# nv-dvl/nerfmatch

Hardware: AMD Instinct MI355X
Metric: rays*samples/sec (higher is better)
Workload: dtype fp16x3 (fp16 MFMA on hi/lo-split fp32 operands, three products per fp32 product, fp32 accumulate; fp32 everywhere else)

## Files before the change

### nerfmatch_amd/csrc/nerf_fwd_bf16.hip

```cpp
#include "nerf_split_chain.h"

namespace {
using namespace nmbf;
using nmsample::HALF_PI_F32, nmsample::SCAN_TILE, nmsample::frustum, nmsample::ray_consts, nmsample::lift_var, nmsample::ipe_fast, nmsample::view_row_value;
using nmsample::alpha_of, nmsample::trans_factor, nmsample::sigmoid, nmsample::scan_before_barrier, nmsample::scan_after_barrier, nmsample::scan_carry;
using nmsample::first_max;
static_assert(TILE == SCAN_TILE, "the compositing scan of nerf_sample.h spans two wavefronts");

template <int PART, bool OWN>
__device__ __forceinline__ void tap_prefetch(Ctx& cx) {
  if constexpr (PART == 0) __builtin_amdgcn_s_barrier();
  const char* src = reinterpret_cast<const char*>(cx.tapw);
#pragma unroll
  for (int q = (PART == 0 ? 0 : 4); q < (PART == 0 ? 4 : 7); ++q) {
    const char* sp = src + q * 4096;
    const float* dp = q < 4 ? cx.tap_ring + q * 1024 : cx.tap_ipe + (q - 4) * 1024;
    const unsigned lds = (unsigned)__builtin_amdgcn_readfirstlane((int)(unsigned)(size_t)(const __attribute__((address_space(3))) float*)dp);
    if constexpr (OWN) {
      asm volatile("s_mov_b32 m0, %0\n\tglobal_load_lds_dwordx4 %1, off\n\tglobal_load_lds_dwordx4 %1, off offset:1024\n\t"
                   "global_load_lds_dwordx4 %1, off offset:2048\n\tglobal_load_lds_dwordx4 %1, off offset:3072"
                   :: "s"(lds), "v"(sp) : "memory");
      continue;
    }
    unsigned m0_saved;
// ... 22 lines not shown
        "v_add_f32_dpp %0, %8, %8 row_half_mirror row_mask:0xf bank_mask:0x5\n\tv_add_f32_dpp %1, %9, %9 row_half_mirror row_mask:0xf bank_mask:0x5\n\t"
        "v_add_f32_dpp %2, %10, %10 row_half_mirror row_mask:0xf bank_mask:0x5\n\tv_add_f32_dpp %3, %11, %11 row_half_mirror row_mask:0xf bank_mask:0x5\n\t"
        "v_add_f32_dpp %4, %12, %12 row_half_mirror row_mask:0xf bank_mask:0x5\n\tv_add_f32_dpp %5, %13, %13 row_half_mirror row_mask:0xf bank_mask:0x5\n\t"
        "v_add_f32_dpp %6, %14, %14 row_half_mirror row_mask:0xf bank_mask:0x5\n\tv_add_f32_dpp %7, %15, %15 row_half_mirror row_mask:0xf bank_mask:0x5\n\t"
        "v_add_f32_dpp %0, %16, %16 row_half_mirror row_mask:0xf bank_mask:0xa\n\tv_add_f32_dpp %1, %17, %17 row_half_mirror row_mask:0xf bank_mask:0xa\n\t"
        "v_add_f32_dpp %2, %18, %18 row_half_mirror row_mask:0xf bank_mask:0xa\n\tv_add_f32_dpp %3, %19, %19 row_half_mirror row_mask:0xf bank_mask:0xa\n\t"
        "v_add_f32_dpp %4, %20, %20 row_half_mirror row_mask:0xf bank_mask:0xa\n\tv_add_f32_dpp %5, %21, %21 row_half_mirror row_mask:0xf bank_mask:0xa\n\t"
        "v_add_f32_dpp %6, %22, %22 row_half_mirror row_mask:0xf bank_mask:0xa\n\tv_add_f32_dpp %7, %23, %23 row_half_mirror row_mask:0xf bank_mask:0xa"
        : "=&v"(o[0]), "=&v"(o[1]), "=&v"(o[2]), "=&v"(o[3]), "=&v"(o[4]), "=&v"(o[5]), "=&v"(o[6]), "=&v"(o[7])
        : "v"(x[0]), "v"(x[1]), "v"(x[2]), "v"(x[3]), "v"(x[4]), "v"(x[5]), "v"(x[6]), "v"(x[7]),
          "v"(y[0]), "v"(y[1]), "v"(y[2]), "v"(y[3]), "v"(y[4]), "v"(y[5]), "v"(y[6]), "v"(y[7]));
}
template <int XOR>
__device__ __forceinline__ void quad_add8(float (&v)[8]) {
  if (XOR == 1)
    asm("s_nop 1\n"
        "v_add_f32_dpp %0, %0, %0 quad_perm:[1,0,3,2] row_mask:0xf bank_mask:0xf\n\tv_add_f32_dpp %1, %1, %1 quad_perm:[1,0,3,2] row_mask:0xf bank_mask:0xf\n\t"
        "v_add_f32_dpp %2, %2, %2 quad_perm:[1,0,3,2] row_mask:0xf bank_mask:0xf\n\tv_add_f32_dpp %3, %3, %3 quad_perm:[1,0,3,2] row_mask:0xf bank_mask:0xf\n\t"
        "v_add_f32_dpp %4, %4, %4 quad_perm:[1,0,3,2] row_mask:0xf bank_mask:0xf\n\tv_add_f32_dpp %5, %5, %5 quad_perm:[1,0,3,2] row_mask:0xf bank_mask:0xf\n\t"
        "v_add_f32_dpp %6, %6, %6 quad_perm:[1,0,3,2] row_mask:0xf bank_mask:0xf\n\tv_add_f32_dpp %7, %7, %7 quad_perm:[1,0,3,2] row_mask:0xf bank_mask:0xf"
        : "+v"(v[0]), "+v"(v[1]), "+v"(v[2]), "+v"(v[3]), "+v"(v[4]), "+v"(v[5]), "+v"(v[6]), "+v"(v[7]));
  else
    asm("s_nop 1\n"
        "v_add_f32_dpp %0, %0, %0 quad_perm:[2,3,0,1] row_mask:0xf bank_mask:0xf\n\tv_add_f32_dpp %1, %1, %1 quad_perm:[2,3,0,1] row_mask:0xf bank_mask:0xf\n\t"
        "v_add_f32_dpp %2, %2, %2 quad_perm:[2,3,0,1] row_mask:0xf bank_mask:0xf\n\tv_add_f32_dpp %3, %3, %3 quad_perm:[2,3,0,1] row_mask:0xf bank_mask:0xf\n\t"
        "v_add_f32_dpp %4, %4, %4 quad_perm:[2,3,0,1] row_mask:0xf bank_mask:0xf\n\tv_add_f32_dpp %5, %5, %5 quad_perm:[2,3,0,1] row_mask:0xf bank_mask:0xf\n\t"
        "v_add_f32_dpp %6, %6, %6 quad_perm:[2,3,0,1] row_mask:0xf bank_mask:0xf\n\tv_add_f32_dpp %7, %7, %7 quad_perm:[2,3,0,1] row_mask:0xf bank_mask:0xf"
        : "+v"(v[0]), "+v"(v[1]), "+v"(v[2]), "+v"(v[3]), "+v"(v[4]), "+v"(v[5]), "+v"(v[6]), "+v"(v[7]));
}
__device__ __forceinline__ float reduce_scatter_step16(float x, float y) {
  const auto r = __builtin_amdgcn_permlane16_swap(__float_as_uint(x), __float_as_uint(y), false, false);
  return __uint_as_float(r[0]) + __uint_as_float(r[1]);
}
__device__ __forceinline__ f32x4 reduce_scatter_16pairs(const float (&s1)[64], int lane) {
  float s2[32];
#pragma unroll
  for (int b = 0; b < 4; ++b) {
    float o[8], x[8], y[8];
#pragma unroll
    for (int i = 0; i < 8; ++i) { x[i] = s1[8 * b + i]; y[i] = s1[32 + 8 * b + i]; }
    dpp_pairs8(o, x, y, true);
#pragma unroll
    for (int i = 0; i < 8; ++i) s2[8 * b + i] = o[i];
  }
  float s3[16];
#pragma unroll
  for (int b = 0; b < 2; ++b) {
    float o[8], x[8], y[8];
#pragma unroll
    for (int i = 0; i < 8; ++i) { x[i] = s2[8 * b + i]; y[i] = s2[16 + 8 * b + i]; }
    dpp_pairs8(o, x, y, false);
#pragma unroll
    for (int i = 0; i < 8; ++i) s3[8 * b + i] = o[i];
  }
  float lo8[8], hi8[8];
#pragma unroll
  for (int i = 0; i < 8; ++i) { lo8[i] = s3[i]; hi8[i] = s3[8 + i]; }
  quad_add8<2>(lo8); quad_add8<2>(hi8);
  float s4[8];
#pragma unroll
  for (int i = 0; i < 8; ++i) s4[i] = (lane & 2) ? hi8[i] : lo8[i];
  float t8[8] = {s4[0], s4[1], s4[2], s4[3], s4[4], s4[5], s4[6], s4[7]};
  quad_add8<1>(t8);
  return (lane & 1) ? f32x4{t8[4], t8[5], t8[6], t8[7]} : f32x4{t8[0], t8[1], t8[2], t8[3]};
}
__device__ __forceinline__ f32x4 reduce_scatter_32rows(float (&v)[128], int lane) {
  float s1[64];
#pragma unroll
  for (int i = 0; i < 64; ++i) s1[i] = reduce_scatter_step16(v[i], v[64 + i]);
  return reduce_scatter_16pairs(s1, lane);
}

#define NM_MLP_DONE_WAIT() __builtin_amdgcn_s_waitcnt(0x0070)
#define NM_EPI_BARRIER() asm volatile("s_waitcnt lgkmcnt(0)\n\ts_barrier" ::: "memory")
template <int P, bool TAP7 = true>
__device__ __forceinline__ void nerf_fwd_body(const NerfArgs& a) {
  constexpr bool DENS = P == 2 && !TAP7;
  __shared__ __attribute__((aligned(16))) float sm[LDS_TOTAL];
  float* const sm_small = sm + LDS_SMALL;
  float* const ring = sm + LDS_RING;
  float* const sm_ipe = sm + LDS_IPE;
  float* const sm_sigma = sm + LDS_SCR;
  float* const sm_rgb = sm_sigma + TILE;
  float* const sm_t0 = sm_rgb + 3 * TILE;
  float* const sm_t1 = sm_t0 + TILE;
  float* const sm_mean = sm_t1 + TILE;
  float* const sm_dn = sm_mean + 3 * TILE;
  float* const sm_w = sm_dn + TILE;
  float* const sm_misc = sm_w + TILE;
  float* const sm_part = sm_misc + 32;
  float* const sm_feat = sm + LDS_FEAT;
  float* const sm_ex = sm + LDS_EX;
  int* const sm_lray = reinterpret_cast<int*>(sm + LDS_LEFT);
  float* const sm_lT = sm + LDS_LEFT + TILE;
  unsigned* const sm_rng = reinterpret_cast<unsigned*>(sm + LDS_RNG);

  const int tid = threadIdx.x, lane = tid & 63, wave = tid >> 6, s = lane & 31, hi = lane >> 5;
  const bool tail_ok = a.left && !(a.tail_viol && *a.tail_viol != 0);
  const int S = a.S, R = a.R;
  const int Sa = tail_ok ? a.Sa : S;
  const int left = tail_ok ? 1 : 0;
  const int ntiles = tail_ok ? a.ntiles : a.ntiles_full;
  const int SP = Sa < TILE ? Sa : TILE;
  const int nr = TILE / SP;
  const int nchunks = (Sa + TILE - 1) / TILE;
  const bool need_rgb = !(a.flags & NM_NERF_SKIP_RGB);
  const bool feat_max = (a.flags & NM_NERF_FEAT_MAX) != 0;
  const bool need_tap = (a.feat != nullptr) || (a.sfeat != nullptr);
  const int tap = (a.tap < 0 || a.tap > 7) ? 7 : a.tap;
  const int nslots = need_rgb ? NSLOT_FULL : NSLOT_NORGB;
  const char* const blob_slots = a.blob + (size_t)SMALL_PAD * 4;

  for (int i = tid; i < SMALL / 4; i += 256) reinterpret_cast<f32x4*>(sm_small)[i] = reinterpret_cast<const f32x4*>(a.blob)[i];
  if constexpr (P == 2) {
#pragma unroll
    for (int k = 0; k < NRANGE; ++k) sm_rng[k * 256 + tid] = 0u;
  }

  int nleft = 0;
  int bid = blockIdx.x;
#pragma unroll 1
  for (;;) {
  bool lo_pass = false;
  if (left && (nleft > TILE - 4 || (bid >= ntiles && nleft > 0))) lo_pass = true;
  else if (bid >= ntiles) break;
  const int nent = lo_pass ? nleft : 0;
  TRACE(0);
  if (need_rgb && !lo_pass && tid < nr * 48) {
    const int r2 = tid / 48, f = tid % 48;
    const int ray2 = bid * nr + r2;
    const float* rq = a.rays + (size_t)(ray2 < R ? ray2 : R - 1) * 12 + 8;
    float v = view_row_value(f, rq[f % 3], a.app_row);
    if constexpr (P == 2) {
      v *= reinterpret_cast<const float*>(a.blob)[OFF_INSCALE + (f < 27 ? 1 : 2)];
      __hip_atomic_fetch_max(sm_rng + 9 * 256 + tid, __float_as_uint(fabsf(v)), __ATOMIC_RELAXED, __HIP_MEMORY_SCOPE_WORKGROUP);
    }
    sm_ex[tid] = v;
  }
  __syncthreads();
// ... 104 lines not shown
          *reinterpret_cast<f32x4*>(sm_part + (tid2 >> 5) * 8) = f32x4{pq[0], pq[1], pq[2], pq[3]};
          *reinterpret_cast<f32x4*>(sm_part + (tid2 >> 5) * 8 + 4) = f32x4{pq[4], pq[5], pq[6], pq[7]};
        }
      }
    };
    auto pick_best = [&]() __attribute__((always_inline)) {
      const int tid2 = launder(threadIdx.x);
      if (tid2 < 8 * nr) {
        const int q = tid2 & 7, r2 = tid2 >> 3;
        const float* wv = sm_w + r2 * SP;
        int bi;
        const bool better = first_max(wv, SP, best_w, bi);
        if (q == 0) sm_misc[8 + r2] = better ? __int_as_float(r2 * SP + bi) : __int_as_float(-1);
        if (q >= 5 && better) red_acc = sm_mean[(q - 5) * TILE + r2 * SP + bi];
      }
    };
    auto tap7_early = [&](Ctx& c) __attribute__((always_inline)) {
      const int t2 = launder(threadIdx.x), jl = (t2 >> 6) * 32 + (t2 & 31), hl = (t2 >> 5) & 1;
      const float sigma_raw = (c.sig_part + nm_shfl_xor32(c.sig_part)) + sm_small[OFF_MISC];
      if (hl == 0) sm_sigma[jl] = sigma_raw;
      NM_EPI_BARRIER();
      composite_weights();
      NM_EPI_BARRIER();
      if (feat_max) {
        pick_best();
        NM_EPI_BARRIER();
      }
      const float desc = sm_small[OFF_DESCALE + 7];
      const float wj = sm_w[jl] * desc;
      const int best = feat_max ? __float_as_int(sm_misc[8 + jl / SP]) : -2;
      const float mult = feat_max ? (jl == best ? desc : 0.f) : wj;
      const float* bl = sm_small + OFF_BIAS + 7 * 256 + 4 * hl;
      const float s7 = sm_small[OFF_SCALE + 7];
      float s1[64];
#pragma unroll
      for (int cq = 0; cq < HS; ++cq) {
        const f32x4 b0 = *reinterpret_cast<const f32x4*>(bl + (cq >> 2) * 32 + 8 * (cq & 3));
        const f32x4 b1 = *reinterpret_cast<const f32x4*>(bl + (4 + (cq >> 2)) * 32 + 8 * (cq & 3));
#pragma unroll
        for (int e = 0; e < 4; ++e) {
          const float x = mult * __builtin_fmaxf(__builtin_fmaf(c.hv[4 * cq + e], s7, b0[e]), 0.f);
          const float y = mult * __builtin_fmaxf(__builtin_fmaf(c.hv[64 + 4 * cq + e], s7, b1[e]), 0.f);
          s1[4 * cq + e] = reduce_scatter_step16(x, y);
        }
      }
      const f32x4 sum4 = reduce_scatter_16pairs(s1, jl);
      const int r = jl & 31;
      float* prow = sm_feat + (jl >> 5) * 256 + 4 * hl;
      *reinterpret_cast<f32x4*>(prow + (r >> 2) * 32 + 16 * ((r >> 1) & 1) + 8 * (r & 1)) = sum4;
    };
    const Tap7InRegisters<decltype(tap7_early)> tap7{early, tap7_early};
    f32x16 acc[8];
    ipe_steps<P, true>(acc, cx, ipe_src);
    finish_layer<P>(acc, 0, cx);
    TRACE(3);
#pragma unroll 1
    for (int l = 1; l < 8; ++l) {
      layer_pass<P, DENS>(acc, l, cx, ipe_src, tap7);
      TRACE(3 + l);
    }
    float c_r = 0.f, c_g = 0.f, c_b = 0.f;
    if (!need_rgb) {
      if (cx.tap == 7) dump_tap(7, cx);
      NM_MLP_DONE_WAIT();
      if (cx.tap_pref) tap_prefetch<0, owns_m0<P>()>(cx);
      alpha_head(cx);
      if (cx.tap_pref) tap_prefetch<1, owns_m0<P>()>(cx);
    } else {
      const int hh = launder(lane) >> 5;
      const float* exr = sm_ex + launder(rl) * 48 + 8 * hh;
      f32x16 av[4];
      if constexpr (DENS) {
        views_hidden<P, true>(av, cx);
        dens_close(cx);
      } else views_hidden<P>(av, cx);
      fold_range<P>(cx, 7);
      bf16x8 exh[VS], exl[VS];
#pragma unroll
      for (int e = 0; e < VS; ++e) {
        float v8[8];
        if (!lo_pass) {
          const f32x4 e0 = *reinterpret_cast<const f32x4*>(exr + 16 * e), e1 = *reinterpret_cast<const f32x4*>(exr + 16 * e + 4);
          v8[0] = e0[0]; v8[1] = e0[1]; v8[2] = e0[2]; v8[3] = e0[3]; v8[4] = e1[0]; v8[5] = e1[1]; v8[6] = e1[2]; v8[7] = e1[3];
        } else {
          const float* rq = a.rays + (size_t)launder(rc) * 12 + 8;
          const float vd0 = rq[0], vd1 = rq[1], vd2 = rq[2];
#pragma unroll
          for (int i = 0; i < 8; ++i) {
            const int f = 16 * e + 8 * hh + i;
            const int ax = f % 3;
            float v = view_row_value(f, ax == 0 ? vd0 : ax == 1 ? vd1 : vd2, a.app_row);
            if constexpr (P == 2) v *= sm_small[OFF_INSCALE + (f < 27 ? 1 : 2)];
            v8[i] = v;
          }
        }
        if constexpr (is_split<P>()) split8_p<P>(v8, exh[e], exl[e]);
        else exh[e] = exl[e] = pack8_f16(v8);
      }
      views_extras<P>(av, cx, exh, exl, a.app_row == nullptr);
      TRACE(11);
      NM_MLP_DONE_WAIT();
      if (cx.tap_pref) tap_prefetch<0, owns_m0<P>()>(cx);
      const float* bv = sm_small + OFF_BVIEWS + 4 * hh;
      const float* wr = sm_small + OFF_WRGB + 4 * hh;
      float pr = 0.f, pg = 0.f, pb = 0.f;
#pragma unroll
      for (int ob = 0; ob < 4; ++ob) {
#pragma unroll
        for (int q = 0; q < 4; ++q) {
          const f32x4 b4 = *reinterpret_cast<const f32x4*>(bv + ob * 32 + 8 * q);
          const f32x4 wr4 = *reinterpret_cast<const f32x4*>(wr + ob * 32 + 8 * q);
          const f32x4 wg4 = *reinterpret_cast<const f32x4*>(wr + 128 + ob * 32 + 8 * q);
          const f32x4 wb4 = *reinterpret_cast<const f32x4*>(wr + 256 + ob * 32 + 8 * q);
#pragma unroll
          for (int e = 0; e < 4; ++e) {
            const float hv = __builtin_fmaxf(acc_read(av[ob][4 * q + e]) + b4[e], 0.f);
            pr = NM_FMA(hv, wr4[e], pr);
            pg = NM_FMA(hv, wg4[e], pg);
            pb = NM_FMA(hv, wb4[e], pb);
          }
        }
      }
      pr = (pr + nm_shfl_xor32(pr)) + sm_small[OFF_MISC + 1];
      pg = (pg + nm_shfl_xor32(pg)) + sm_small[OFF_MISC + 2];
      pb = (pb + nm_shfl_xor32(pb)) + sm_small[OFF_MISC + 3];
      c_r = sigmoid(pr);
      c_g = sigmoid(pg);
      c_b = sigmoid(pb);
      if (cx.tap_pref) tap_prefetch<1, owns_m0<P>()>(cx);
    }
    const float sigma_raw = (cx.sig_part + nm_shfl_xor32(cx.sig_part)) + sm_small[OFF_MISC];
    TRACE(12);
    {
      const int jsw = launder(js);
      if ((launder(lane) >> 5) == 0) {
// ... 240 lines not shown
```

### nerfmatch_amd/csrc/nerf_split_chain.h

```cpp
#pragma once
#include "nerf_bf16_common.h"

namespace nmbf {

template <int P> constexpr bool is_bf16() { return P == 0 || P == 3 || P == 4; }
template <int P> constexpr bool has_gates() { return P == 4; }
typedef _Float16 f16x8 __attribute__((ext_vector_type(8)));
typedef _Float16 f16x2 __attribute__((ext_vector_type(2)));
template <int P>
__device__ __forceinline__ f32x16 mfma_p(const bf16x8& a, const bf16x8& b, const f32x16& c) {
  if constexpr (is_bf16<P>()) return MFMA_BF16(a, b, c);
  else return __builtin_amdgcn_mfma_f32_32x32x16_f16(__builtin_bit_cast(f16x8, a), __builtin_bit_cast(f16x8, b), c, 0, 0, 0);
}
template <int P> constexpr bool is_split() { return P != 1; }
template <int P> constexpr int slot_bytes() { return is_split<P>() ? SLOT_BYTES : SLOT_BYTES / 2; }
template <int P> constexpr int slot_floats() { return slot_bytes<P>() / 4; }
template <int P> constexpr int ring_slots() { return is_split<P>() ? NRING : 2 * NRING; }
template <int P> constexpr int ring_ahead() { return is_split<P>() ? 4 : 6; }
constexpr float F16_MAX = 65504.0f;
__device__ __forceinline__ void split8_f16(const float (&v)[8], bf16x8& hi, bf16x8& lo) {
  f16x8 h8, l8;
#pragma unroll
  for (int i = 0; i < 8; ++i) {
    const float c = __builtin_amdgcn_fmed3f(v[i], -F16_MAX, F16_MAX);
// ... 195 lines not shown
#pragma unroll
  for (int g0 = 0; g0 < (is_split<P>() ? 2 : ring_ahead<P>()); ++g0) dma_slot<P>(blob_slots, g0, ring, wave, lane);
}
template <int P>
__device__ __forceinline__ void ring_open_wait(Ctx& cx) {
  cx.dma_voff = (unsigned)(cx.wave * (slot_bytes<P>() / 4) + cx.lane * 16);
  const float* q = cx.ring + cx.wave * (slot_floats<P>() / 4);
  const unsigned lds0 = (unsigned)__builtin_amdgcn_readfirstlane((int)(unsigned)(size_t)(const __attribute__((address_space(3))) float*)q);
  if constexpr (owns_m0<P>()) {
    cx.dma_m = lds0; cx.dma_s = 2u * lds0 + 2u * (unsigned)slot_bytes<P>();
    cx.dma_p = (unsigned long long)(size_t)(cx.blob_slots + slot_bytes<P>());
    cx.dma_q = cx.dma_p;
  } else {
    cx.dma_lds = lds0;
  }
  NM_WAIT_VMCNT(0);
  __builtin_amdgcn_s_barrier();
}

__device__ __forceinline__ unsigned gate_byte(const u32x4& h) {
  const unsigned w0 = h[0], w1 = h[1], w2 = h[2], w3 = h[3];
  unsigned m0, m1, m2, m3;
  const unsigned one = 0x00010001u;
  asm("v_pk_min_u16 %0, %1, %2" : "=v"(m0) : "v"(w0), "v"(one));
  asm("v_pk_min_u16 %0, %1, %2" : "=v"(m1) : "v"(w1), "v"(one));
  asm("v_pk_min_u16 %0, %1, %2" : "=v"(m2) : "v"(w2), "v"(one));
  asm("v_pk_min_u16 %0, %1, %2" : "=v"(m3) : "v"(w3), "v"(one));
  const unsigned t = m0 | (m1 << 1) | (m2 << 2) | (m3 << 3);
  return (t & 0xfu) | ((t >> 12) & 0xf0u);
}

template <bool BF, class W> __device__ __forceinline__ void unit_seq(W& w, int c);
template <bool EVEN, bool BF, class W> __device__ __forceinline__ void unit_step8(W& w, int t);
template <int P, bool DENS = false>
struct UnitWork {
  Ctx& cx;
  Unit& out;
  int u, lo_;
  float floor_v;
  f32x4 b0, b1;
  float sc;
  float v8[8];
  float f0, f1;
  float r0[4], r1[4];
  f32x4 wa0, wa1;
  __device__ __forceinline__ static void dens_fma(float& p, float v, float w) { asm volatile("v_fma_f32 %0, %1, %2, %0" : "+v"(p) : "v"(v), "v"(w)); }
  __device__ __forceinline__ void dens_seq(int c) {
    if constexpr (DENS) {
      switch (c) {
        case 0: {
          const float* wl = cx.sm_small + OFF_WALPHA + (u >> 1) * 32 + 16 * (u & 1) + 4 * cx.hi;
          wa0 = *reinterpret_cast<const f32x4*>(wl); wa1 = *reinterpret_cast<const f32x4*>(wl + 8);
        } break;
        case 1:
          dens_fma(cx.dp[1], cx.dv[0], cx.dw[0]); dens_fma(cx.dp[2], cx.dv[1], cx.dw[1]); dens_fma(cx.dp[3], cx.dv[2], cx.dw[2]);
          break;
        case 7: dens_fma(cx.dp[0], v8[0], wa0[0]); break;
        case 10: dens_fma(cx.dp[0], v8[4], wa1[0]); break;
        case 11:
          dens_fma(cx.dp[1], v8[1], wa0[1]); dens_fma(cx.dp[2], v8[2], wa0[2]); dens_fma(cx.dp[3], v8[3], wa0[3]);
          cx.dv[0] = v8[5]; cx.dw[0] = wa1[1]; cx.dv[1] = v8[6]; cx.dw[1] = wa1[2]; cx.dv[2] = v8[7]; cx.dw[2] = wa1[3];
          break;
        default: break;
      }
    }
  }
  __device__ __forceinline__ void bias() {
    if constexpr (P == 2) {
      b0 = cx.nb0; b1 = cx.nb1;
      return;
    }
    const int ob = u >> 1, m = u & 1;
    const float* bl = cx.sm_small + OFF_BIAS + lo_ * 256 + ob * 32 + 16 * m + 4 * cx.hi;
    b0 = *reinterpret_cast<const f32x4*>(bl); b1 = *reinterpret_cast<const f32x4*>(bl + 8);
  }
  __device__ __forceinline__ void bias_next() {
    if constexpr (P == 2) {
      if (u + 1 < HS) {
        const int ob = (u + 1) >> 1, m = (u + 1) & 1;
        const float* bl = cx.sm_small + OFF_BIAS + lo_ * 256 + ob * 32 + 16 * m + 4 * cx.hi;
        cx.nb0 = *reinterpret_cast<const f32x4*>(bl); cx.nb1 = *reinterpret_cast<const f32x4*>(bl + 8);
      }
    }
  }
  __device__ __forceinline__ float act(int e, float b) const {
    const float h = cx.hv[(u >> 1) * 16 + 8 * (u & 1) + e];
    if constexpr (is_bf16<P>()) return __builtin_fmaxf(h + b, floor_v);
    else if constexpr (P == 1) return __builtin_amdgcn_fmed3f(h + b, floor_v, F16_MAX);
    else return __builtin_amdgcn_fmed3f(__builtin_fmaf(h, sc, b), floor_v, F16_MAX);
  }
  __device__ __forceinline__ void range(int j) {
    if constexpr (P == 2) asm("v_max3_f32 %0, |%1|, |%2|, %0" : "+v"(cx.vmax) : "v"(v8[j]), "v"(v8[4 + j]));
  }
  __device__ __forceinline__ void ra(int j) { v8[j] = act(j, b0[j]); pin(v8[j]); }
  __device__ __forceinline__ void rb(int j) { v8[4 + j] = act(4 + j, b1[j]); range(j); pin(v8[4 + j]); }
  __device__ __forceinline__ void relu(int j) {
    v8[j] = act(j, b0[j]); v8[4 + j] = act(4 + j, b1[j]);
    range(j);
    pin(v8[j]); pin(v8[4 + j]);
  }
  __device__ __forceinline__ void hi(int p) {
    unsigned hp;
    if constexpr (is_bf16<P>()) {
      hp = pack_bf16(v8[2 * p], v8[2 * p + 1]);
      f0 = __uint_as_float(hp << 16);
      f1 = __uint_as_float(hp & 0xffff0000u);
    } else {
      hp = pack_f16(v8[2 * p], v8[2 * p + 1]);
    }
    pin(hp);
    if constexpr (is_bf16<P>()) { pin(f0); pin(f1); }
    out.h[p] = hp;
  }
  __device__ __forceinline__ void rem(int p) {
    if constexpr (is_bf16<P>()) {
      r0[p] = v8[2 * p] - f0; r1[p] = v8[2 * p + 1] - f1;
      pin(r0[p]); pin(r1[p]);
    } else {
      asm volatile("v_fma_mix_f32 %0, %1, -1.0, %2 op_sel:[0,0,0] op_sel_hi:[1,0,0]" : "=v"(r0[p]) : "v"(out.h[p]), "v"(v8[2 * p]));
      asm volatile("v_fma_mix_f32 %0, %1, -1.0, %2 op_sel:[1,0,0] op_sel_hi:[1,0,0]" : "=v"(r1[p]) : "v"(out.h[p]), "v"(v8[2 * p + 1]));
    }
  }
  __device__ __forceinline__ void lo(int p) {
    unsigned lp = is_bf16<P>() ? pack_bf16(r0[p], r1[p]) : pack_f16(r0[p], r1[p]);
    pin(lp);
    out.l[p] = lp;
  }
  __device__ __forceinline__ void gates() {
    if constexpr (has_gates<P>()) {
      const unsigned t = gate_byte(out.h);
      cx.gbits[u >> 2] |= t << (8 * (u & 3));
    }
// ... 95 lines not shown
  for (int k = 0; k < s; ++k) n += take_n(k);
  return n;
}
constexpr int TAKE_HIDDEN = take_before(12);
__device__ __forceinline__ const float* unit0_bias(const Ctx& cx, int l) { return cx.sm_small + OFF_BIAS + l * 256 + 4 * cx.hi; }
template <int P>
struct AccTake {
  const f32x16 (&acc)[8];
  Ctx& cx;
  int l;
  __device__ __forceinline__ void prefetch() {}
  __device__ __forceinline__ void operator()(int j) {
#pragma unroll
    for (int k = 0; k < 8; ++k) {
      const int i = 8 * j + k;
      if (i < 64) cx.hv[i] = acc_read(acc[i >> 4][i & 15]);
    }
  }
  __device__ __forceinline__ void seq(int) {}
  template <bool EVEN> __device__ __forceinline__ void step8(int t) {
    if (t < 12) return;
    const int s = t - 12;
#pragma unroll
    for (int k = 0; k < take_n(s); ++k) {
      const int i = take_before(s) + k;
      cx.hv[i] = acc_read(acc[i >> 4][i & 15]);
    }
    if (s == 10) {
      const float* bl = unit0_bias(cx, l);
      cx.hb0 = *reinterpret_cast<const f32x4*>(bl); cx.hb1 = *reinterpret_cast<const f32x4*>(bl + 8);
    }
  }
};
template <int P, bool DENS = false>
__device__ __forceinline__ UnitWork<P, DENS> unit_work(int u, int lo, Ctx& cx, Unit& out) {
  return UnitWork<P, DENS>{cx, out, u, lo, lo < 8 ? 0.f : (!is_bf16<P>() ? -F16_MAX : -__builtin_inff()), {}, {}, cx.sc, {}, 0.f, 0.f, {}, {}, {}, {}};
}

template <int P>
__device__ __forceinline__ void finish_layer(const f32x16 (&acc)[8], int l, Ctx& cx) {
  if constexpr (is_split<P>()) {
#pragma unroll
    for (int i = TAKE_HIDDEN; i < 64; ++i) cx.hv[i] = acc_read(acc[i >> 4][i & 15]);
  }
#pragma unroll
  for (int ob = 4; ob < 8; ++ob)
#pragma unroll
    for (int r = 0; r < 16; ++r) cx.hv[ob * 16 + r] = acc_read(acc[ob][r]);
  if constexpr (P == 2)
    cx.sc = __builtin_bit_cast(float, __builtin_amdgcn_readfirstlane(__builtin_bit_cast(int, cx.sm_small[OFF_SCALE + l])));
  UnitWork<P> w = unit_work<P>(0, l, cx, cx.xn);
  if constexpr (P == 2) {
    const float* bl = unit0_bias(cx, l) + 16;
    cx.nb0 = *reinterpret_cast<const f32x4*>(bl); cx.nb1 = *reinterpret_cast<const f32x4*>(bl + 8);
  }
  if constexpr (is_split<P>()) {
    w.b0 = cx.hb0; w.b1 = cx.hb1;
#pragma unroll
    for (int j = 0; j < 4; ++j) w.relu(j);
#pragma unroll
    for (int p = 0; p < 4; ++p) {
      w.hi(p);
      if constexpr (is_bf16<P>()) w.rem(p);
    }
    if constexpr (!is_bf16<P>()) {
#pragma unroll
      for (int p = 0; p < 4; ++p) w.rem(p);
    }
#pragma unroll
    for (int p = 0; p < 4; ++p) w.lo(p);
    w.gates();
  } else {
    w.prefetch();
#pragma unroll
    for (int j = 0; j < 12; ++j) w(j);
  }
}

__device__ __forceinline__ void alpha_head(Ctx& cx) {
  const float* bl = cx.sm_small + OFF_BIAS + 7 * 256 + 4 * cx.hi;
  const float* wa = cx.sm_small + OFF_WALPHA + 4 * cx.hi;
  const float s7 = cx.sm_small[OFF_SCALE + 7];
  float p0 = 0.f, p1 = 0.f, p2 = 0.f, p3 = 0.f;
#pragma unroll
  for (int ob = 0; ob < 8; ++ob)
#pragma unroll
    for (int q = 0; q < 4; ++q) {
      const f32x4 b = *reinterpret_cast<const f32x4*>(bl + ob * 32 + 8 * q);
      const f32x4 w4v = *reinterpret_cast<const f32x4*>(wa + ob * 32 + 8 * q);
      p0 = NM_FMA(__builtin_fmaxf(__builtin_fmaf(cx.hv[ob * 16 + 4 * q + 0], s7, b[0]), 0.f), w4v[0], p0);
      p1 = NM_FMA(__builtin_fmaxf(__builtin_fmaf(cx.hv[ob * 16 + 4 * q + 1], s7, b[1]), 0.f), w4v[1], p1);
      p2 = NM_FMA(__builtin_fmaxf(__builtin_fmaf(cx.hv[ob * 16 + 4 * q + 2], s7, b[2]), 0.f), w4v[2], p2);
      p3 = NM_FMA(__builtin_fmaxf(__builtin_fmaf(cx.hv[ob * 16 + 4 * q + 3], s7, b[3]), 0.f), w4v[3], p3);
    }
  cx.sig_part = (p0 + p1) + (p2 + p3);
}

__device__ __forceinline__ void dens_open(Ctx& cx) {
  const float* bl = cx.sm_small + OFF_BIAS + 7 * 256 + 4 * cx.hi;
  const float* wa = cx.sm_small + OFF_WALPHA + 4 * cx.hi;
  const f32x4 b0 = *reinterpret_cast<const f32x4*>(bl), b1 = *reinterpret_cast<const f32x4*>(bl + 8);
  const f32x4 w0 = *reinterpret_cast<const f32x4*>(wa), w1 = *reinterpret_cast<const f32x4*>(wa + 8);
  float v[8];
#pragma unroll
  for (int j = 0; j < 4; ++j) {
    v[j] = __builtin_fmaxf(__builtin_fmaf(cx.hv[j], cx.sc, b0[j]), 0.f);
    v[4 + j] = __builtin_fmaxf(__builtin_fmaf(cx.hv[4 + j], cx.sc, b1[j]), 0.f);
  }
#pragma unroll
  for (int j = 0; j < 4; ++j) cx.dp[j] = NM_FMA(v[j], w0[j], 0.f);
  cx.dp[0] = NM_FMA(v[4], w1[0], cx.dp[0]);
#pragma unroll
  for (int j = 0; j < 3; ++j) { cx.dv[j] = v[5 + j]; cx.dw[j] = w1[1 + j]; }
}
struct DensTail {
  Ctx& cx;
  __device__ __forceinline__ void seq(int c) {
    if (c == 1) {
#pragma unroll
      for (int j = 0; j < 3; ++j) UnitWork<2, true>::dens_fma(cx.dp[1 + j], cx.dv[j], cx.dw[j]);
    }
  }
};
__device__ __forceinline__ void dens_close(Ctx& cx) { cx.sig_part = (cx.dp[0] + cx.dp[1]) + (cx.dp[2] + cx.dp[3]); }

__device__ __forceinline__ void dump_tap(int lo, Ctx& cx) {
  const float* bl = cx.sm_small + OFF_BIAS + lo * 256 + 4 * cx.hi;
  const float sl = cx.sm_small[OFF_SCALE + lo];
  auto* tp = (__attribute__((address_space(1))) f32x4*)cx.tapw;
#pragma unroll
  for (int ob = 0; ob < 8; ++ob) {
    f32x4 v[4];
#pragma unroll
    for (int q = 0; q < 4; ++q) {
      const f32x4 b = *reinterpret_cast<const f32x4*>(bl + ob * 32 + 8 * q);
#pragma unroll
      for (int e = 0; e < 4; ++e) v[q][e] = __builtin_fmaxf(__builtin_fmaf(cx.hv[ob * 16 + 4 * q + e], sl, b[e]), 0.f);
    }
#pragma unroll
    for (int q = 0; q < 4; ++q) tp[q * 64] = v[q];
    tp += 256;
    pin(tp);
  }
}

__device__ __forceinline__ bf16x8 load_op1(const float* slot, int lane, int blk) {
  return __builtin_bit_cast(bf16x8, (reinterpret_cast<const u32x4*>(slot) + lane)[blk * 64]);
}
#define NM_SB __builtin_amdgcn_sched_barrier(0)
template <bool FIRST, bool ACQ, class Work>
__device__ __forceinline__ void slot_step8_one(f32x16 (&acc)[8], Ctx& cx, const bf16x8& x, Work work) {
  const f32x16 zero = {0.f, 0.f, 0.f, 0.f, 0.f, 0.f, 0.f, 0.f, 0.f, 0.f, 0.f, 0.f, 0.f, 0.f, 0.f, 0.f};
  const int g = cx.g;
  const OpHalf A = cx.opA, B = cx.opB;
  const float* nxt = ring_slot<1>(cx.ring, g + 1);
  acc[0] = mfma_p<1>(A.h[0], x, FIRST ? zero : acc[0]); NM_SB;
  if constexpr (ACQ) ring_acquire_pair(cx.blob_slots, g, cx.ring, cx.wave, cx.lane);
  NM_SB;
  acc[1] = mfma_p<1>(A.h[1], x, FIRST ? zero : acc[1]); NM_SB;
  cx.opA.h[0] = load_op1(nxt, cx.lane, 0); cx.opA.h[1] = load_op1(nxt, cx.lane, 1); work.prefetch(); NM_SB;
  acc[2] = mfma_p<1>(A.h[2], x, FIRST ? zero : acc[2]); NM_SB;
  cx.opA.h[2] = load_op1(nxt, cx.lane, 2); cx.opA.h[3] = load_op1(nxt, cx.lane, 3); NM_SB;
  acc[3] = mfma_p<1>(A.h[3], x, FIRST ? zero : acc[3]); NM_SB;
  cx.opB.h[0] = load_op1(nxt, cx.lane, 4); cx.opB.h[1] = load_op1(nxt, cx.lane, 5); NM_SB;
  acc[4] = mfma_p<1>(B.h[0], x, FIRST ? zero : acc[4]); NM_SB;
  cx.opB.h[2] = load_op1(nxt, cx.lane, 6); cx.opB.h[3] = load_op1(nxt, cx.lane, 7); NM_SB;
  acc[5] = mfma_p<1>(B.h[1], x, FIRST ? zero : acc[5]); NM_SB;
// ... 120 lines not shown
  OpHalf B;
  const float* cur = cx.ring + (g & (NRING - 1)) * SLOT_FLOATS;
  const float* nxt = cx.ring + ((g + 1) & (NRING - 1)) * SLOT_FLOATS;
#pragma unroll
  for (int k = 0; k < 12; ++k) {
    av[k & 3] = mfma_k<P, FIRST>(k, A, x0h, x0l, av[k & 3]);
    __builtin_amdgcn_sched_barrier(0);
    if (k >= 1 && k <= 4) load_pair<P>(B, cur, cx.lane, 1, k - 1);
    if constexpr (EVEN) {
      if (k == 0 || k == 2) ring_arm<P>(cx, k >> 1);
      if (k >= 4) ring_request<P>(cx, g, k - 4);
    }
    if (k == 11) lds_retire<P>();
    w0.seq(k);
    __builtin_amdgcn_sched_barrier(0);
  }
  if constexpr (!EVEN) {
    ring_acquire_two();
    __builtin_amdgcn_sched_barrier(0);
  }
  const bf16x8 x1h = __builtin_bit_cast(bf16x8, u1.h), x1l = __builtin_bit_cast(bf16x8, u1.l);
#pragma unroll
  for (int k = 0; k < 12; ++k) {
    av[k & 3] = mfma_k<P, false>(k, B, x1h, x1l, av[k & 3]);
    __builtin_amdgcn_sched_barrier(0);
    if (k >= 1 && k <= 4) load_pair<P>(cx.opA, nxt, cx.lane, 0, k - 1);
    if (k == 11) lds_retire<P>();
    w1.seq(k);
    __builtin_amdgcn_sched_barrier(0);
  }
  cx.g = g + 1;
}

template <int P, bool DENS = false>
__device__ __forceinline__ void views_hidden(f32x16 (&av)[4], Ctx& cx) {
  static_assert(!DENS || P == 2, "the density head accumulates in the views K-loop in fp16x3 only");
  if constexpr (is_split<P>()) {
#pragma unroll
    for (int sl = 0; sl < HS / 2; ++sl) {
      const Unit x0 = cx.xn;
      Unit u1;
      const bf16x8 x0h = __builtin_bit_cast(bf16x8, x0.h), x0l = __builtin_bit_cast(bf16x8, x0.l);
      if (sl == 0) slot_step4x2<P, true, true>(av, cx, x0h, x0l, u1, unit_work<P, DENS>(1, 7, cx, u1), unit_work<P, DENS>(2, 7, cx, cx.xn));
      else if (sl + 1 == HS / 2) {
        if constexpr (DENS) slot_step4x2<P, false, false>(av, cx, x0h, x0l, u1, unit_work<P, DENS>(2 * sl + 1, 7, cx, u1), DensTail{cx});
        else slot_step4x2<P, false, false>(av, cx, x0h, x0l, u1, unit_work<P>(2 * sl + 1, 7, cx, u1), NoWork{});
      } else if (sl & 1) slot_step4x2<P, false, false>(av, cx, x0h, x0l, u1, unit_work<P, DENS>(2 * sl + 1, 7, cx, u1), unit_work<P, DENS>(2 * sl + 2, 7, cx, cx.xn));
      else slot_step4x2<P, false, true>(av, cx, x0h, x0l, u1, unit_work<P, DENS>(2 * sl + 1, 7, cx, u1), unit_work<P, DENS>(2 * sl + 2, 7, cx, cx.xn));
    }
  } else {
#pragma unroll
    for (int ks = 0; ks < HS; ks += 2) {
      {
        const Unit xc = cx.xn;
        if (ks == 0) slot_step4<P, true, true>(av, cx, __builtin_bit_cast(bf16x8, xc.h), __builtin_bit_cast(bf16x8, xc.l), unit_work<P>(ks + 1, 7, cx, cx.xn));
        else slot_step4<P, false, true>(av, cx, __builtin_bit_cast(bf16x8, xc.h), __builtin_bit_cast(bf16x8, xc.l), unit_work<P>(ks + 1, 7, cx, cx.xn));
      }
      {
        const Unit xc = cx.xn;
        if (ks + 2 < HS) slot_step4<P, false, false>(av, cx, __builtin_bit_cast(bf16x8, xc.h), __builtin_bit_cast(bf16x8, xc.l), unit_work<P>(ks + 2, 7, cx, cx.xn));
        else slot_step4<P, false, false>(av, cx, __builtin_bit_cast(bf16x8, xc.h), __builtin_bit_cast(bf16x8, xc.l), NoWork{});
      }
    }
  }
}
template <int P>
__device__ __forceinline__ void views_extras(f32x16 (&av)[4], Ctx& cx, const bf16x8 (&eh)[VS], const bf16x8 (&el)[VS], bool no_app) {
  if constexpr (is_split<P>()) {
    Unit u1;
    u1.h = __builtin_bit_cast(u32x4, eh[1]); u1.l = __builtin_bit_cast(u32x4, el[1]);
    slot_step4x2<P, false, true>(av, cx, eh[0], el[0], u1, NoWork{}, NoWork{});
    if (!no_app) slot_step4<P, false, false>(av, cx, eh[2], el[2], NoWork{});
  } else {
    slot_step4<P, false, true>(av, cx, eh[0], el[0], NoWork{});
    slot_step4<P, false, false>(av, cx, eh[1], el[1], NoWork{});
    if (!no_app) slot_step4<P, false, true>(av, cx, eh[2], el[2], NoWork{});
  }
}

template <int P, bool FIRST>
__device__ __forceinline__ void ipe_steps(f32x16 (&acc)[8], Ctx& cx, const float* ipe_src, int l = FIRST ? 0 : 5) {
// ... 6 lines not shown
    bf16x8 ph, pl, qh, ql;
    operand(0, ph, pl);
#pragma unroll
    for (int m = 0; m < XS; m += 2) {
      if (m == 0) slot_step8<P, FIRST, true>(acc, cx, ph, pl, IpeFetch<17>{ipe_src, m + 1, qh, ql});
      else slot_step8<P, false, true, true>(acc, cx, ph, pl, IpeFetch<6>{ipe_src, m + 1, qh, ql});
      if (m + 2 == XS) slot_step8<P, false, false>(acc, cx, qh, ql, AccTake<P>{acc, cx, l});
      else slot_step8<P, false, false, true>(acc, cx, qh, ql, IpeFetch<4>{ipe_src, m + 2, ph, pl});
    }
    return;
  }
#pragma unroll
  for (int m = 0; m < XS; m += 2) {
    bf16x8 ph, pl;
    operand(m, ph, pl);
    if (m == 0) slot_step8<P, FIRST, true>(acc, cx, ph, pl, NoWork{});
    else slot_step8<P, false, true>(acc, cx, ph, pl, NoWork{});
    operand(m + 1, ph, pl);
    if (m + 2 == XS) slot_step8<P, false, false>(acc, cx, ph, pl, AccTake<P>{acc, cx, l});
    else slot_step8<P, false, false>(acc, cx, ph, pl, NoWork{});
  }
}

struct Tap7Workspace {
  static constexpr bool on = false;
  __device__ __forceinline__ void fn(Ctx&) const {}
};
template <class F>
struct Tap7InRegisters {
  bool on;
  F fn;
};

template <int P, bool DENS = false, class Tap7 = Tap7Workspace>
__device__ __forceinline__ void layer_pass(f32x16 (&acc)[8], int l, Ctx& cx, const float* ipe_src, const Tap7& tap7 = Tap7()) {
  if (l - 1 == cx.tap) dump_tap(l - 1, cx);
#pragma unroll
  for (int ks = 0; ks < HS; ks += 2) {
    {
      const Unit xc = cx.xn;
      if (ks == 0) slot_step8<P, true, true>(acc, cx, __builtin_bit_cast(bf16x8, xc.h), __builtin_bit_cast(bf16x8, xc.l), unit_work<P>(ks + 1, l - 1, cx, cx.xn));
      else slot_step8<P, false, true, request_early<P>()>(acc, cx, __builtin_bit_cast(bf16x8, xc.h), __builtin_bit_cast(bf16x8, xc.l), unit_work<P>(ks + 1, l - 1, cx, cx.xn));
    }
    {
      const Unit xc = cx.xn;
      if (ks + 2 < HS) slot_step8<P, false, false, request_early<P>()>(acc, cx, __builtin_bit_cast(bf16x8, xc.h), __builtin_bit_cast(bf16x8, xc.l), unit_work<P>(ks + 2, l - 1, cx, cx.xn));
      else slot_step8<P, false, false>(acc, cx, __builtin_bit_cast(bf16x8, xc.h), __builtin_bit_cast(bf16x8, xc.l), AccTake<P>{acc, cx, l});
    }
  }
  fold_range<P>(cx, l - 1);
  if constexpr (has_gates<P>()) {
    cx.gptr[(l - 1) * 256] = u32x4{cx.gbits[0], cx.gbits[1], cx.gbits[2], cx.gbits[3]};
    cx.gbits[0] = cx.gbits[1] = cx.gbits[2] = cx.gbits[3] = 0u;
  }
  if (l == 5) ipe_steps<P, false>(acc, cx, ipe_src);
  finish_layer<P>(acc, l, cx);
  if (l == 7) {
    if (cx.rgb) {
      if (cx.tap == 7 && !tap7.on) dump_tap(7, cx);
      if constexpr (DENS) dens_open(cx);
      else alpha_head(cx);
      if (tap7.on) tap7.fn(cx);
    }
  }
}

}
```

Before: 401.1 million.

## Defer layer-7 tap compositing behind the views K-loop using kept activations

For the fp16x3 form with tap 7 enabled, the density head now rides the views K-loop (DENS) and the layer-7 tap dump and compositing are moved after the views MLP. They reuse activated hidden values stored in cx.hv by the unit work and dens_open, so bias/ReLU is not recomputed. The intent is to take the tap-7 barriers and compositing work off the critical path before the views layer and overlap it with later work. In exchange, need_rgb is forced on in this path and the kept activations add register pressure.

```diff
diff --git a/nerfmatch_amd/csrc/nerf_fwd_bf16.hip b/nerfmatch_amd/csrc/nerf_fwd_bf16.hip
--- a/nerfmatch_amd/csrc/nerf_fwd_bf16.hip
+++ b/nerfmatch_amd/csrc/nerf_fwd_bf16.hip
@@ -78,17 +78,7 @@
   const auto r = __builtin_amdgcn_permlane16_swap(__float_as_uint(x), __float_as_uint(y), false, false);
   return __uint_as_float(r[0]) + __uint_as_float(r[1]);
 }
-__device__ __forceinline__ f32x4 reduce_scatter_16pairs(const float (&s1)[64], int lane) {
-  float s2[32];
-#pragma unroll
-  for (int b = 0; b < 4; ++b) {
-    float o[8], x[8], y[8];
-#pragma unroll
-    for (int i = 0; i < 8; ++i) { x[i] = s1[8 * b + i]; y[i] = s1[32 + 8 * b + i]; }
-    dpp_pairs8(o, x, y, true);
-#pragma unroll
-    for (int i = 0; i < 8; ++i) s2[8 * b + i] = o[i];
-  }
+__device__ __forceinline__ f32x4 reduce_scatter_8pairs(const float (&s2)[32], int lane) {
   float s3[16];
 #pragma unroll
   for (int b = 0; b < 2; ++b) {
@@ -110,6 +100,19 @@
   quad_add8<1>(t8);
   return (lane & 1) ? f32x4{t8[4], t8[5], t8[6], t8[7]} : f32x4{t8[0], t8[1], t8[2], t8[3]};
 }
+__device__ __forceinline__ f32x4 reduce_scatter_16pairs(const float (&s1)[64], int lane) {
+  float s2[32];
+#pragma unroll
+  for (int b = 0; b < 4; ++b) {
+    float o[8], x[8], y[8];
+#pragma unroll
+    for (int i = 0; i < 8; ++i) { x[i] = s1[8 * b + i]; y[i] = s1[32 + 8 * b + i]; }
+    dpp_pairs8(o, x, y, true);
+#pragma unroll
+    for (int i = 0; i < 8; ++i) s2[8 * b + i] = o[i];
+  }
+  return reduce_scatter_8pairs(s2, lane);
+}
 __device__ __forceinline__ f32x4 reduce_scatter_32rows(float (&v)[128], int lane) {
   float s1[64];
 #pragma unroll
@@ -121,7 +124,8 @@
 #define NM_EPI_BARRIER() asm volatile("s_waitcnt lgkmcnt(0)\n\ts_barrier" ::: "memory")
 template <int P, bool TAP7 = true>
 __device__ __forceinline__ void nerf_fwd_body(const NerfArgs& a) {
-  constexpr bool DENS = P == 2 && !TAP7;
+  constexpr bool DENS = P == 2;
+  constexpr bool LATE7 = P == 2 && TAP7;
   __shared__ __attribute__((aligned(16))) float sm[LDS_TOTAL];
   float* const sm_small = sm + LDS_SMALL;
   float* const ring = sm + LDS_RING;
@@ -150,7 +154,7 @@
   const int SP = Sa < TILE ? Sa : TILE;
   const int nr = TILE / SP;
   const int nchunks = (Sa + TILE - 1) / TILE;
-  const bool need_rgb = !(a.flags & NM_NERF_SKIP_RGB);
+  const bool need_rgb = LATE7 || !(a.flags & NM_NERF_SKIP_RGB);
   const bool feat_max = (a.flags & NM_NERF_FEAT_MAX) != 0;
   const bool need_tap = (a.feat != nullptr) || (a.sfeat != nullptr);
   const int tap = (a.tap < 0 || a.tap > 7) ? 7 : a.tap;
@@ -321,31 +325,49 @@
       const float mult = feat_max ? (jl == best ? desc : 0.f) : wj;
       const float* bl = sm_small + OFF_BIAS + 7 * 256 + 4 * hl;
       const float s7 = sm_small[OFF_SCALE + 7];
-      float s1[64];
-#pragma unroll
-      for (int cq = 0; cq < HS; ++cq) {
-        const f32x4 b0 = *reinterpret_cast<const f32x4*>(bl + (cq >> 2) * 32 + 8 * (cq & 3));
-        const f32x4 b1 = *reinterpret_cast<const f32x4*>(bl + (4 + (cq >> 2)) * 32 + 8 * (cq & 3));
-#pragma unroll
-        for (int e = 0; e < 4; ++e) {
-          const float x = mult * __builtin_fmaxf(__builtin_fmaf(c.hv[4 * cq + e], s7, b0[e]), 0.f);
-          const float y = mult * __builtin_fmaxf(__builtin_fmaf(c.hv[64 + 4 * cq + e], s7, b1[e]), 0.f);
-          s1[4 * cq + e] = reduce_scatter_step16(x, y);
-        }
-      }
-      const f32x4 sum4 = reduce_scatter_16pairs(s1, jl);
+      f32x4 sum4;
+      if constexpr (LATE7) {
+        float s2[32];
+#pragma unroll
+        for (int b = 0; b < 4; ++b) {
+          float o[8], x[8], y[8];
+#pragma unroll
+          for (int i = 0; i < 8; ++i) {
+            x[i] = reduce_scatter_step16(mult * c.hv[8 * b + i], mult * c.hv[64 + 8 * b + i]);
+            y[i] = reduce_scatter_step16(mult * c.hv[32 + 8 * b + i], mult * c.hv[96 + 8 * b + i]);
+          }
+          dpp_pairs8(o, x, y, true);
+#pragma unroll
+          for (int i = 0; i < 8; ++i) s2[8 * b + i] = o[i];
+        }
+        sum4 = reduce_scatter_8pairs(s2, jl);
+      } else {
+        float s1[64];
+#pragma unroll
+        for (int cq = 0; cq < HS; ++cq) {
+          const f32x4 b0 = *reinterpret_cast<const f32x4*>(bl + (cq >> 2) * 32 + 8 * (cq & 3));
+          const f32x4 b1 = *reinterpret_cast<const f32x4*>(bl + (4 + (cq >> 2)) * 32 + 8 * (cq & 3));
+#pragma unroll
+          for (int e = 0; e < 4; ++e) {
+            const float x = mult * __builtin_fmaxf(__builtin_fmaf(c.hv[4 * cq + e], s7, b0[e]), 0.f);
+            const float y = mult * __builtin_fmaxf(__builtin_fmaf(c.hv[64 + 4 * cq + e], s7, b1[e]), 0.f);
+            s1[4 * cq + e] = reduce_scatter_step16(x, y);
+          }
+        }
+        sum4 = reduce_scatter_16pairs(s1, jl);
+      }
       const int r = jl & 31;
       float* prow = sm_feat + (jl >> 5) * 256 + 4 * hl;
       *reinterpret_cast<f32x4*>(prow + (r >> 2) * 32 + 16 * ((r >> 1) & 1) + 8 * (r & 1)) = sum4;
     };
-    const Tap7InRegisters<decltype(tap7_early)> tap7{early, tap7_early};
+    const Tap7InRegisters<decltype(tap7_early)> tap7{early && !LATE7, tap7_early};
     f32x16 acc[8];
     ipe_steps<P, true>(acc, cx, ipe_src);
     finish_layer<P>(acc, 0, cx);
     TRACE(3);
 #pragma unroll 1
     for (int l = 1; l < 8; ++l) {
-      layer_pass<P, DENS>(acc, l, cx, ipe_src, tap7);
+      layer_pass<P, DENS, LATE7>(acc, l, cx, ipe_src, tap7);
       TRACE(3 + l);
     }
     float c_r = 0.f, c_g = 0.f, c_b = 0.f;
@@ -360,7 +382,7 @@
       const float* exr = sm_ex + launder(rl) * 48 + 8 * hh;
       f32x16 av[4];
       if constexpr (DENS) {
-        views_hidden<P, true>(av, cx);
+        views_hidden<P, true, LATE7>(av, cx);
         dens_close(cx);
       } else views_hidden<P>(av, cx);
       fold_range<P>(cx, 7);
@@ -388,8 +410,14 @@
       }
       views_extras<P>(av, cx, exh, exl, a.app_row == nullptr);
       TRACE(11);
+      if constexpr (LATE7) {
+        if (cx.tap == 7 && !early) dump_tap<true>(7, cx);
+      }
       NM_MLP_DONE_WAIT();
       if (cx.tap_pref) tap_prefetch<0, owns_m0<P>()>(cx);
+      if constexpr (LATE7) {
+        if (early) tap7_early(cx);
+      }
       const float* bv = sm_small + OFF_BVIEWS + 4 * hh;
       const float* wr = sm_small + OFF_WRGB + 4 * hh;
       float pr = 0.f, pg = 0.f, pb = 0.f;
diff --git a/nerfmatch_amd/csrc/nerf_split_chain.h b/nerfmatch_amd/csrc/nerf_split_chain.h
--- a/nerfmatch_amd/csrc/nerf_split_chain.h
+++ b/nerfmatch_amd/csrc/nerf_split_chain.h
@@ -251,7 +251,7 @@
 
 template <bool BF, class W> __device__ __forceinline__ void unit_seq(W& w, int c);
 template <bool EVEN, bool BF, class W> __device__ __forceinline__ void unit_step8(W& w, int t);
-template <int P, bool DENS = false>
+template <int P, bool DENS = false, bool KEEP = false>
 struct UnitWork {
   Ctx& cx;
   Unit& out;
@@ -311,12 +311,16 @@
   __device__ __forceinline__ void range(int j) {
     if constexpr (P == 2) asm("v_max3_f32 %0, |%1|, |%2|, %0" : "+v"(cx.vmax) : "v"(v8[j]), "v"(v8[4 + j]));
   }
-  __device__ __forceinline__ void ra(int j) { v8[j] = act(j, b0[j]); pin(v8[j]); }
-  __device__ __forceinline__ void rb(int j) { v8[4 + j] = act(4 + j, b1[j]); range(j); pin(v8[4 + j]); }
+  __device__ __forceinline__ void keep(int e) {
+    if constexpr (KEEP) cx.hv[(u >> 1) * 16 + 8 * (u & 1) + e] = v8[e];
+  }
+  __device__ __forceinline__ void ra(int j) { v8[j] = act(j, b0[j]); pin(v8[j]); keep(j); }
+  __device__ __forceinline__ void rb(int j) { v8[4 + j] = act(4 + j, b1[j]); range(j); pin(v8[4 + j]); keep(4 + j); }
   __device__ __forceinline__ void relu(int j) {
     v8[j] = act(j, b0[j]); v8[4 + j] = act(4 + j, b1[j]);
     range(j);
     pin(v8[j]); pin(v8[4 + j]);
+    keep(j); keep(4 + j);
   }
   __device__ __forceinline__ void hi(int p) {
     unsigned hp;
@@ -478,9 +482,9 @@
     }
   }
 };
-template <int P, bool DENS = false>
-__device__ __forceinline__ UnitWork<P, DENS> unit_work(int u, int lo, Ctx& cx, Unit& out) {
-  return UnitWork<P, DENS>{cx, out, u, lo, lo < 8 ? 0.f : (!is_bf16<P>() ? -F16_MAX : -__builtin_inff()), {}, {}, cx.sc, {}, 0.f, 0.f, {}, {}, {}, {}};
+template <int P, bool DENS = false, bool KEEP = false>
+__device__ __forceinline__ UnitWork<P, DENS, KEEP> unit_work(int u, int lo, Ctx& cx, Unit& out) {
+  return UnitWork<P, DENS, KEEP>{cx, out, u, lo, lo < 8 ? 0.f : (!is_bf16<P>() ? -F16_MAX : -__builtin_inff()), {}, {}, cx.sc, {}, 0.f, 0.f, {}, {}, {}, {}};
 }
 
 template <int P>
@@ -542,6 +546,7 @@
   cx.sig_part = (p0 + p1) + (p2 + p3);
 }
 
+template <bool KEEP = false>
 __device__ __forceinline__ void dens_open(Ctx& cx) {
   const float* bl = cx.sm_small + OFF_BIAS + 7 * 256 + 4 * cx.hi;
   const float* wa = cx.sm_small + OFF_WALPHA + 4 * cx.hi;
@@ -553,6 +558,10 @@
     v[j] = __builtin_fmaxf(__builtin_fmaf(cx.hv[j], cx.sc, b0[j]), 0.f);
     v[4 + j] = __builtin_fmaxf(__builtin_fmaf(cx.hv[4 + j], cx.sc, b1[j]), 0.f);
   }
+  if constexpr (KEEP) {
+#pragma unroll
+    for (int j = 0; j < 8; ++j) cx.hv[j] = v[j];
+  }
 #pragma unroll
   for (int j = 0; j < 4; ++j) cx.dp[j] = NM_FMA(v[j], w0[j], 0.f);
   cx.dp[0] = NM_FMA(v[4], w1[0], cx.dp[0]);
@@ -570,6 +579,7 @@
 };
 __device__ __forceinline__ void dens_close(Ctx& cx) { cx.sig_part = (cx.dp[0] + cx.dp[1]) + (cx.dp[2] + cx.dp[3]); }
 
+template <bool ACT = false>
 __device__ __forceinline__ void dump_tap(int lo, Ctx& cx) {
   const float* bl = cx.sm_small + OFF_BIAS + lo * 256 + 4 * cx.hi;
   const float sl = cx.sm_small[OFF_SCALE + lo];
@@ -579,6 +589,11 @@
     f32x4 v[4];
 #pragma unroll
     for (int q = 0; q < 4; ++q) {
+      if constexpr (ACT) {
+#pragma unroll
+        for (int e = 0; e < 4; ++e) v[q][e] = cx.hv[ob * 16 + 4 * q + e];
+        continue;
+      }
       const f32x4 b = *reinterpret_cast<const f32x4*>(bl + ob * 32 + 8 * q);
 #pragma unroll
       for (int e = 0; e < 4; ++e) v[q][e] = __builtin_fmaxf(__builtin_fmaf(cx.hv[ob * 16 + 4 * q + e], sl, b[e]), 0.f);
@@ -765,21 +780,22 @@
   cx.g = g + 1;
 }
 
-template <int P, bool DENS = false>
+template <int P, bool DENS = false, bool KEEP = false>
 __device__ __forceinline__ void views_hidden(f32x16 (&av)[4], Ctx& cx) {
   static_assert(!DENS || P == 2, "the density head accumulates in the views K-loop in fp16x3 only");
+  static_assert(!KEEP || DENS, "activated values are kept by the form whose density head rides the views K-loop");
   if constexpr (is_split<P>()) {
 #pragma unroll
     for (int sl = 0; sl < HS / 2; ++sl) {
       const Unit x0 = cx.xn;
       Unit u1;
       const bf16x8 x0h = __builtin_bit_cast(bf16x8, x0.h), x0l = __builtin_bit_cast(bf16x8, x0.l);
-      if (sl == 0) slot_step4x2<P, true, true>(av, cx, x0h, x0l, u1, unit_work<P, DENS>(1, 7, cx, u1), unit_work<P, DENS>(2, 7, cx, cx.xn));
+      if (sl == 0) slot_step4x2<P, true, true>(av, cx, x0h, x0l, u1, unit_work<P, DENS, KEEP>(1, 7, cx, u1), unit_work<P, DENS, KEEP>(2, 7, cx, cx.xn));
       else if (sl + 1 == HS / 2) {
-        if constexpr (DENS) slot_step4x2<P, false, false>(av, cx, x0h, x0l, u1, unit_work<P, DENS>(2 * sl + 1, 7, cx, u1), DensTail{cx});
+        if constexpr (DENS) slot_step4x2<P, false, false>(av, cx, x0h, x0l, u1, unit_work<P, DENS, KEEP>(2 * sl + 1, 7, cx, u1), DensTail{cx});
         else slot_step4x2<P, false, false>(av, cx, x0h, x0l, u1, unit_work<P>(2 * sl + 1, 7, cx, u1), NoWork{});
-      } else if (sl & 1) slot_step4x2<P, false, false>(av, cx, x0h, x0l, u1, unit_work<P, DENS>(2 * sl + 1, 7, cx, u1), unit_work<P, DENS>(2 * sl + 2, 7, cx, cx.xn));
-      else slot_step4x2<P, false, true>(av, cx, x0h, x0l, u1, unit_work<P, DENS>(2 * sl + 1, 7, cx, u1), unit_work<P, DENS>(2 * sl + 2, 7, cx, cx.xn));
+      } else if (sl & 1) slot_step4x2<P, false, false>(av, cx, x0h, x0l, u1, unit_work<P, DENS, KEEP>(2 * sl + 1, 7, cx, u1), unit_work<P, DENS, KEEP>(2 * sl + 2, 7, cx, cx.xn));
+      else slot_step4x2<P, false, true>(av, cx, x0h, x0l, u1, unit_work<P, DENS, KEEP>(2 * sl + 1, 7, cx, u1), unit_work<P, DENS, KEEP>(2 * sl + 2, 7, cx, cx.xn));
     }
   } else {
 #pragma unroll
@@ -852,7 +868,7 @@
   F fn;
 };
 
-template <int P, bool DENS = false, class Tap7 = Tap7Workspace>
+template <int P, bool DENS = false, bool LATE7 = false, class Tap7 = Tap7Workspace>
 __device__ __forceinline__ void layer_pass(f32x16 (&acc)[8], int l, Ctx& cx, const float* ipe_src, const Tap7& tap7 = Tap7()) {
   if (l - 1 == cx.tap) dump_tap(l - 1, cx);
 #pragma unroll
@@ -877,12 +893,17 @@
   finish_layer<P>(acc, l, cx);
   if (l == 7) {
     if (cx.rgb) {
-      if (cx.tap == 7 && !tap7.on) dump_tap(7, cx);
-      if constexpr (DENS) dens_open(cx);
-      else alpha_head(cx);
-      if (tap7.on) tap7.fn(cx);
-    }
-  }
-}
-
-}
+      if constexpr (LATE7) {
+        static_assert(DENS, "a tap composited behind the views K-loop takes its weights from the density head that rides it");
+        dens_open<true>(cx);
+      } else {
+        if (cx.tap == 7 && !tap7.on) dump_tap(7, cx);
+        if constexpr (DENS) dens_open(cx);
+        else alpha_head(cx);
+        if (tap7.on) tap7.fn(cx);
+      }
+    }
+  }
+}
+
+}
```

After: 404.0 million (median of 5 runs). No clear change (+0.7%).
